# schwanbeck/YSMR

Hardware: AMD Instinct MI355X
Metric: frames/sec detect+link, 1228x922 ~500 blobs, 1/2/4/8 GPU; HBM GB/s %peak (higher is better)
Workload: dtype u8 image / f32 threshold+geometry / f64 link; 1 GPU; 1228x922 stream, ~500 blobs, detect+link end to end (BASELINE configs[2], the configuration the metric is quoted on); detect_batch=248, channels=1, streams=1, parallelism=1 stream/GPU x1, tracks_alive=508, ids_issued=796

## Files before the change

### ysmr_amd/csrc/batch_link.h

```cpp
#pragma once

#include "tracker_plan.h"

constexpr unsigned BL_FLAG = 0xFFFFu, BL_SPLIT = 0xFFFEu;

constexpr int BG_THREADS = 256, BG_PER = 10;
constexpr int BG_CAND = 32;
static_assert(BG_THREADS == 4 * 64 && BL_OVF <= 64, "k_bgrid's second pass: quadrant w of overflow entry `lane` on wave w");
static_assert(BG_THREADS * BG_PER >= FUSED_MAX_DET, "k_bgrid keeps a frame's detections in registers, BG_PER per thread");

__device__ __forceinline__ void bl_rect_list(int cx, int cy, float ax, float bx, float ay, float by, float e, int G, int m, float cell,
                                             float inv, const unsigned short *start16, const float2 *xy, unsigned short *list8,
                                             unsigned short *cand)
{
    float u2 = 3.0e38f;
    int ju = 0;
    auto far2 = [&](int a, int b) {
        for (int j = a; j < b; ++j) {
            const float2 d = xy[j];
            const float dx = fmaxf(fabsf(d.x - ax), fabsf(d.x - bx)), dy = fmaxf(fabsf(d.y - ay), fabsf(d.y - by));
            const float v = dx * dx + dy * dy;
            ju = v < u2 ? j : ju;
            u2 = fminf(u2, v);
        }
    };
    for (int r = 0; r < G; ++r) {
        const int xl = max(cx - r, 0), xh = min(cx + r, G - 1);
        for (int y = max(cy - r, 0); y <= min(cy + r, G - 1); ++y) {
            if (y == cy - r || y == cy + r) far2(start16[y * G + xl], start16[y * G + xh + 1]);
            else {
                if (cx - r >= 0) far2(start16[y * G + cx - r], start16[y * G + cx - r + 1]);
                if (cx + r < G) far2(start16[y * G + cx + r], start16[y * G + cx + r + 1]);
            }
        }
        const float reach = (float)(r + 1) * cell;
        if (u2 <= reach * reach) break;
    }
    const float T = sqrtf(u2) * 1.0001f + 1.0f, T2 = T * T;
    const int rho = min((int)((T + e) * inv) + 2, G);
    int n = 0;
    for (int y = max(cy - rho, 0); y <= min(cy + rho, G - 1); ++y) {
        const int a = start16[y * G + max(cx - rho, 0)], b = start16[y * G + min(cx + rho, G - 1) + 1];
        for (int j = a; j < b; ++j) {
            const float2 d = xy[j];
            const float dx = fmaxf(fmaxf(ax - d.x, d.x - bx), 0.f), dy = fmaxf(fmaxf(ay - d.y, d.y - by), 0.f);
            if (dx * dx + dy * dy <= T2) {
                if (n < BG_CAND) cand[n * BG_THREADS] = (unsigned short)j;
                ++n;
            }
        }
    }
    int kept = 0;
    const float2 du = xy[ju];
    const float ua = ax - du.x, ub = bx - du.x, va = ay - du.y, vb = by - du.y;
    const float eps = 1.00003f, beta = 0.6f;
    const float u0 = (ua * ua + va * va) * eps + beta, u1 = (ub * ub + va * va) * eps + beta;
    const float u2c = (ua * ua + vb * vb) * eps + beta, u3 = (ub * ub + vb * vb) * eps + beta;
    if (n <= BG_CAND)
        for (int i = 0; i < n; ++i) {
            const int ji = cand[i * BG_THREADS];
            const float2 di = xy[ji];
            const float xa = ax - di.x, xb = bx - di.x, ya = ay - di.y, yb = by - di.y;
            const float s0 = xa * xa + ya * ya, s1 = xb * xb + ya * ya, s2 = xa * xa + yb * yb, s3 = xb * xb + yb * yb;
            bool beaten = ji != ju && s0 > u0 && s1 > u1 && s2 > u2c && s3 > u3;
            for (int k = 0; k < n && !beaten; k += 4) {
                float2 dk[4];
#pragma unroll
                for (int u = 0; u < 4; ++u) dk[u] = xy[cand[min(k + u, n - 1) * BG_THREADS]];
#pragma unroll
                for (int u = 0; u < 4; ++u) {
                    const float ka = ax - dk[u].x, kb = bx - dk[u].x, la = ay - dk[u].y, lb = by - dk[u].y;
                    beaten = beaten || (k + u < n && k + u != i && s0 > (ka * ka + la * la) * eps + beta && s1 > (kb * kb + la * la) * eps + beta &&
                                        s2 > (ka * ka + lb * lb) * eps + beta && s3 > (kb * kb + lb * lb) * eps + beta);
                }
            }
            if (!beaten) {
                if (kept < BL_LIST) list8[kept] = (unsigned short)ji;
                ++kept;
            }
        }
    if (n > BG_CAND || kept > BL_LIST) list8[0] = (unsigned short)BL_FLAG;
    else
        for (int k = kept; k < BL_LIST; ++k) list8[k] = (unsigned short)m;
}
__device__ __forceinline__ void bl_cell_list(int c, int G, int m, float x0, float y0, float cell, float inv, const unsigned short *start16,
                                             const float2 *xy, unsigned short *list16, unsigned short *cand)
{
    const int cx = c % G, cy = c / G;
    const float e = 4e-3f + 2e-4f * cell;
    const float ax = x0 + (float)cx * cell - e, bx = x0 + (float)(cx + 1) * cell + e;
    const float ay = y0 + (float)cy * cell - e, by = y0 + (float)(cy + 1) * cell + e;
    bl_rect_list(cx, cy, ax, bx, ay, by, e, G, m, cell, inv, start16, xy, list16 + c * BL_LIST, cand);
}
__device__ __forceinline__ void bl_quad_list(int c, int q, int G, int m, float x0, float y0, float cell, float inv, const unsigned short *start16,
                                             const float2 *xy, unsigned short *list8, unsigned short *cand)
{
    const int cx = c % G, cy = c / G;
    const float e = 4e-3f + 2e-4f * cell;
    const float hx = (float)cx + 0.5f * (float)(q & 1), hy = (float)cy + 0.5f * (float)(q >> 1);
    const float ax = x0 + hx * cell - e, bx = x0 + (hx + 0.5f) * cell + e;
    const float ay = y0 + hy * cell - e, by = y0 + (hy + 0.5f) * cell + e;
    bl_rect_list(cx, cy, ax, bx, ay, by, e, G, m, cell, inv, start16, xy, list8, cand);
}

template <bool D3>
__device__ __forceinline__ void bl_bin_frame(const float *__restrict__ det_all, const double *__restrict__ third_all,
                                             const int32_t *__restrict__ det_count, int max_det, char *grid, unsigned grid_stride)
{
    extern __shared__ __attribute__((aligned(16))) uint32_t s_out[];
    __shared__ int s_cnt[64 * 64];
    __shared__ float s_red[4][4];
    __shared__ int s_wave_sum[4];
    const int f = blockIdx.x, tid = threadIdx.x, lane = tid & 63, w = tid >> 6;
    __shared__ unsigned short s_cand[BG_CAND][BG_THREADS];
    __shared__ unsigned short s_crowded[BL_OVF];
    __shared__ int s_crowded_n;
    __shared__ int s_any_crowded;
    __shared__ int s_wide;
    const float *det = det_all + (size_t)f * max_det * 5;
    int m = det_count[f];
    m = m < 0 ? 0 : (m > max_det ? max_det : m);
    const int G = bl_grid_n(m), cells = G * G;
    unsigned short *start16 = reinterpret_cast<unsigned short *>(s_out + 16);
    float2 *xy = reinterpret_cast<float2 *>(s_out + 16 + bl_start_dwords(G));
    unsigned short *items = reinterpret_cast<unsigned short *>(s_out + 16 + bl_start_dwords(G) + 2 * bl_mp(m));
    unsigned short *list16 = reinterpret_cast<unsigned short *>(s_out + bl_list_off(m));
    float *z32 = reinterpret_cast<float *>(s_out + bl_list_off(m));
    double *z64 = nullptr;
    if constexpr (D3) z64 = reinterpret_cast<double *>(grid + (size_t)grid_stride * f + 4 * (size_t)bl3_lds_dwords_max(max_det));
    float x[BG_PER], y[BG_PER];
    double z[BG_PER];
    bool wide = false;
#pragma unroll
    for (int k = 0; k < BG_PER; ++k) {
        const int j = tid + k * BG_THREADS;
        x[k] = j < m ? det[(size_t)j * 5] : 0.f;
        y[k] = j < m ? det[(size_t)j * 5 + 1] : 0.f;
        if constexpr (D3) {
            z[k] = j < m ? (third_all + (size_t)f * max_det)[j] : 0.0;
            wide = wide || !(fabs(z[k]) < 4096.0);
        }
    }
    for (int c = tid; c < cells; c += BG_THREADS) s_cnt[c] = 0;
    if constexpr (D3) { if (tid == 0) s_wide = 0; }
    float lo_x = 3.0e38f, lo_y = 3.0e38f, hi_x = -3.0e38f, hi_y = -3.0e38f;
#pragma unroll
    for (int k = 0; k < BG_PER; ++k)
        if (tid + k * BG_THREADS < m) { lo_x = fminf(lo_x, x[k]); hi_x = fmaxf(hi_x, x[k]); lo_y = fminf(lo_y, y[k]); hi_y = fmaxf(hi_y, y[k]); }
#pragma unroll
    for (int d = 32; d >= 1; d >>= 1) {
        lo_x = fminf(lo_x, __shfl_xor(lo_x, d)); hi_x = fmaxf(hi_x, __shfl_xor(hi_x, d));
        lo_y = fminf(lo_y, __shfl_xor(lo_y, d)); hi_y = fmaxf(hi_y, __shfl_xor(hi_y, d));
    }
    if (lane == 0) { s_red[0][w] = lo_x; s_red[1][w] = hi_x; s_red[2][w] = lo_y; s_red[3][w] = hi_y; }
    __syncthreads();
    if constexpr (D3) { if (wide) s_wide = 1; }
    lo_x = s_red[0][0]; hi_x = s_red[1][0]; lo_y = s_red[2][0]; hi_y = s_red[3][0];
    for (int k = 1; k < 4; ++k) {
        lo_x = fminf(lo_x, s_red[0][k]); hi_x = fmaxf(hi_x, s_red[1][k]);
        lo_y = fminf(lo_y, s_red[2][k]); hi_y = fmaxf(hi_y, s_red[3][k]);
    }
    if (m == 0) { lo_x = lo_y = 0.f; hi_x = hi_y = 1.f; }
    const float extent = fmaxf(fmaxf(hi_x - lo_x, hi_y - lo_y), 1.0f);
    const float cell = extent / (float)(G - 2), inv = 1.0f / cell;
    const float x0 = lo_x - cell, y0 = lo_y - cell;
    if (tid < 16) s_out[tid] = 0;
    __syncthreads();
    if (tid == 0) {
        float *h = reinterpret_cast<float *>(s_out);
        h[0] = x0; h[1] = y0; h[2] = cell; h[3] = inv;
        s_out[4] = (uint32_t)G; s_out[5] = (uint32_t)m; s_out[6] = !D3 && bl_has_lists(m) ? BL_LIST : 0;
        if constexpr (D3) s_out[7] = (uint32_t)s_wide;
    }
    int cell_of[BG_PER];
#pragma unroll
    for (int k = 0; k < BG_PER; ++k) {
        int cx = (int)floorf((x[k] - x0) * inv), cy = (int)floorf((y[k] - y0) * inv);
        cx = cx < 0 ? 0 : (cx > G - 1 ? G - 1 : cx);
        cy = cy < 0 ? 0 : (cy > G - 1 ? G - 1 : cy);
        cell_of[k] = cy * G + cx;
        if (tid + k * BG_THREADS < m) atomicAdd(&s_cnt[cell_of[k]], 1);
    }
    __syncthreads();
    const int K = cells / BG_THREADS;
    int local[16], sum = 0;
#pragma unroll
    for (int k = 0; k < 16; ++k)
        if (k < K) { local[k] = sum; sum += s_cnt[tid * K + k]; }
    int incl = sum;
#pragma unroll
    for (int d = 1; d < 64; d <<= 1) { const int o = __shfl_up(incl, d); if (lane >= d) incl += o; }
    if (lane == 63) s_wave_sum[w] = incl;
    __syncthreads();
    int before = incl - sum;
    for (int k = 0; k < w; ++k) before += s_wave_sum[k];
#pragma unroll
    for (int k = 0; k < 16; ++k)
        if (k < K) {
            const int at = before + local[k];
            s_cnt[tid * K + k] = at;
            start16[tid * K + k] = (unsigned short)at;
        }
    if (tid == BG_THREADS - 1) { start16[cells] = (unsigned short)m; start16[cells + 1] = 0; }
    for (int j = m + tid; j < bl_mp(m); j += BG_THREADS) {
        xy[j] = make_float2(1.0e30f, 1.0e30f); items[j] = 0;
        if constexpr (D3) { z32[j] = 0.f; z64[j] = 0.0; }
    }
    __syncthreads();
#pragma unroll
    for (int k = 0; k < BG_PER; ++k) {
        const int j = tid + k * BG_THREADS;
        if (j < m) {
            const int at = atomicAdd(&s_cnt[cell_of[k]], 1);
            items[at] = (unsigned short)j;
            xy[at] = make_float2(x[k], y[k]);
            if constexpr (D3) { z32[at] = (float)z[k]; z64[at] = z[k]; }
        }
    }
    if (!D3 && bl_has_lists(m)) {
        for (int i = tid; i < BL_OVF * 4 * BL_LIST / 2; i += BG_THREADS) s_out[bl_ovf_off(m) + i] = 0;
        if (tid == 0) s_any_crowded = 0;
    }
    __syncthreads();
    if constexpr (!D3) {
        unsigned short *ovf16 = reinterpret_cast<unsigned short *>(s_out + bl_ovf_off(m));
        if (bl_has_lists(m) && m > 0) {
            for (int c = tid; c < cells; c += BG_THREADS) {
                bl_cell_list(c, G, m, x0, y0, cell, inv, start16, xy, list16, &s_cand[0][tid]);
                if (list16[c * BL_LIST] == BL_FLAG) s_any_crowded = 1;
            }
            __syncthreads();
        }
        if (bl_has_lists(m) && m > 0 && s_any_crowded) {
            int mine = 0;
#pragma unroll
            for (int k = 0; k < 16; ++k)
                if (k < K) mine += list16[(tid * K + k) * BL_LIST] == BL_FLAG;
            int inc2 = mine;
#pragma unroll
            for (int d = 1; d < 64; d <<= 1) { const int o = __shfl_up(inc2, d); if (lane >= d) inc2 += o; }
            if (lane == 63) s_wave_sum[w] = inc2;
            __syncthreads();
            int at = inc2 - mine;
            for (int k = 0; k < w; ++k) at += s_wave_sum[k];
            if (mine)
                for (int k = 0; k < K; ++k)
                    if (list16[(tid * K + k) * BL_LIST] == BL_FLAG) {
                        if (at < BL_OVF) s_crowded[at] = (unsigned short)(tid * K + k);
                        ++at;
                    }
            if (tid == BG_THREADS - 1) s_crowded_n = min(at, BL_OVF);
            __syncthreads();
            const int entries = s_crowded_n;
            if (lane < entries)
                bl_quad_list(s_crowded[lane], w, G, m, x0, y0, cell, inv, start16, xy, ovf16 + (4 * lane + w) * BL_LIST, &s_cand[0][tid]);
            __syncthreads();
            if (tid < entries) {
                bool fits = true;
                for (int q = 0; q < 4; ++q) fits = fits && ovf16[(4 * tid + q) * BL_LIST] != BL_FLAG;
                if (fits) reinterpret_cast<uint32_t *>(list16)[s_crowded[tid] * (BL_LIST / 2)] = BL_SPLIT | ((uint32_t)tid << 16);
            }
            __syncthreads();
        }
    }
    uint4 *out = reinterpret_cast<uint4 *>(grid + (size_t)grid_stride * f);
    const uint4 *img = reinterpret_cast<const uint4 *>(s_out);
    for (int i = tid; i < (D3 ? bl3_lds_dwords(m) : bl_grid_dwords(m)) / 4; i += BG_THREADS) out[i] = img[i];
}

__global__ __launch_bounds__(BG_THREADS) void k_bgrid(const float *__restrict__ det_all, const int32_t *__restrict__ det_count,
                                                      int max_det, char *grid, unsigned grid_stride)
{
    bl_bin_frame<false>(det_all, nullptr, det_count, max_det, grid, grid_stride);
}

struct BlSeat {
    double s0x[BL_NF], s1x[BL_NF], s0y[BL_NF], s1y[BL_NF];
    double w[BL_NF], xa[BL_NF], xb[BL_NF];
    double px, py;
    float info[3];
    int id, gone, len, mode, rank;
    bool alive;
};

__device__ __forceinline__ void bl_seat_blank(BlSeat &S)
{
#pragma unroll
    for (int f = 0; f < BL_NF; ++f) { S.s0x[f] = S.s1x[f] = S.s0y[f] = S.s1y[f] = 0.0; S.w[f] = S.xa[f] = S.xb[f] = 0.0; }
    S.px = S.py = 0.0;
    S.info[0] = S.info[1] = S.info[2] = 0.f;
    S.id = S.gone = S.len = S.mode = S.rank = 0;
    S.alive = false;
}

__device__ __forceinline__ void bl_seat_load(BlSeat &S, const BatchDev &bd, int at)
{
    const size_t sc = (size_t)bd.seat_cap;
    const double *p = bd.f64 + at;
#pragma unroll
    for (int f = 0; f < BL_NF; ++f) { S.w[f] = p[sc * f]; S.xa[f] = p[sc * (BL_NF + f)]; S.xb[f] = p[sc * (2 * BL_NF + f)]; }
    S.px = p[sc * (3 * BL_NF)];
    S.py = p[sc * (3 * BL_NF + 1)];
#pragma unroll
    for (int f = 0; f < BL_NF; ++f) {
        const double *q = p + sc * (3 * BL_NF + 2 + 4 * f);
        S.s0x[f] = q[0]; S.s1x[f] = q[sc]; S.s0y[f] = q[2 * sc]; S.s1y[f] = q[3 * sc];
    }
#pragma unroll
    for (int k = 0; k < 3; ++k) S.info[k] = bd.f32[sc * k + at];
    S.id = bd.i32[at]; S.gone = bd.i32[sc + at]; S.len = bd.i32[2 * sc + at]; S.mode = bd.i32[3 * sc + at];
    S.rank = bd.i32[4 * sc + at];
}

__device__ __forceinline__ void bl_seat_store(const BlSeat &S, const BatchDev &bd, int at)
{
    const size_t sc = (size_t)bd.seat_cap;
    double *p = bd.f64 + at;
#pragma unroll
    for (int f = 0; f < BL_NF; ++f) { p[sc * f] = S.w[f]; p[sc * (BL_NF + f)] = S.xa[f]; p[sc * (2 * BL_NF + f)] = S.xb[f]; }
    p[sc * (3 * BL_NF)] = S.px;
    p[sc * (3 * BL_NF + 1)] = S.py;
#pragma unroll
    for (int f = 0; f < BL_NF; ++f) {
        double *q = p + sc * (3 * BL_NF + 2 + 4 * f);
        q[0] = S.s0x[f]; q[sc] = S.s1x[f]; q[2 * sc] = S.s0y[f]; q[3 * sc] = S.s1y[f];
    }
// ... 1317 lines not shown
    const int span = cap > bd.seat_cap ? cap : bd.seat_cap;
    for (int s = blockIdx.x * blockDim.x + threadIdx.x; s < span; s += gridDim.x * blockDim.x) {
        if (s < cap - n) d.free_slots[s] = cap - 1 - s;
        if (s == 0) *d.n_free = cap - n;
        if (s >= bd.seat_cap || n == 0 || !bd.i32[5 * sc + s]) continue;
        const int r = bd.i32[4 * sc + s];
        const double *p = bd.f64 + s;
        double *hist = d.hist + (size_t)r * 2 * L;
        for (int e = 0; e < L && e < BL_HB - 1; ++e) {
            const double2 v = bd.ring[(size_t)((head - 1 - e) & (BL_HB - 1)) * sc + s];
            hist[2 * e] = v.x; hist[2 * e + 1] = v.y;
        }
        double *rec = d.rec + (size_t)r * d.rec_stride;
        rec[0] = __longlong_as_double((long long)(unsigned int)bd.i32[2 * sc + s]);
        rec[1] = __longlong_as_double((long long)(unsigned int)bd.i32[3 * sc + s]);
        for (int f = 0; f < nf && f < BL_NF; ++f) {
            rec[2 + f] = p[sc * f];
            rec[2 + nf + f] = p[sc * (BL_NF + f)];
            rec[2 + 2 * nf + f] = p[sc * (2 * BL_NF + f)];
        }
        d.pos[r] = p[sc * (3 * BL_NF)];
        d.pos[cap + r] = p[sc * (3 * BL_NF + 1)];
        if (seat3) pos3[r] = seat3[s];
        for (int k = 0; k < 3; ++k) d.info[k * cap + r] = bd.f32[sc * k + s];
        d.id[r] = bd.i32[s];
        d.order[r] = r;
        d.gone[r] = bd.i32[sc + s];
        d.row_gone[r] = bd.i32[sc + s];
    }
}

__global__ void k_peek_batch(TrackerDev t, BatchDev bd, int32_t *ids, double *xy, int32_t *gone, int32_t *n_out)
{
    const size_t sc = (size_t)bd.seat_cap;
    const int s = blockIdx.x * blockDim.x + threadIdx.x;
    const int n = *t.n_tracks;
    if (s == 0 && n_out) *n_out = n;
    if (s >= bd.seat_cap || n == 0 || !bd.i32[5 * sc + s]) return;
    const int i = bd.i32[4 * sc + s];
    if (ids) ids[i] = bd.i32[s];
    if (xy) { xy[2 * i] = bd.f64[sc * (3 * BL_NF) + s]; xy[2 * i + 1] = bd.f64[sc * (3 * BL_NF + 1) + s]; }
    if (gone) gone[i] = bd.i32[sc + s];
}

__global__ void k_peek_third_batch(TrackerDev t, BatchDev bd, const double *seat3, double *third)
{
    const size_t sc = (size_t)bd.seat_cap;
    const int s = blockIdx.x * blockDim.x + threadIdx.x;
    if (s >= bd.seat_cap || *t.n_tracks == 0 || !bd.i32[5 * sc + s]) return;
    third[bd.i32[4 * sc + s]] = seat3[s];
}


__global__ __launch_bounds__(BG_THREADS) void k_bgrid3(const float *__restrict__ det_all, const double *__restrict__ third_all,
                                                       const int32_t *__restrict__ det_count, int max_det, char *grid, unsigned grid_stride)
{
    bl_bin_frame<true>(det_all, third_all, det_count, max_det, grid, grid_stride);
}

struct Bl3Seat {
    double px, py, pz;
    float info[3];
    int id, gone, rank;
    bool alive;
};

struct BlKernArgs3 {
    TrackerDev t;
    BatchDev bd;
    const float *det_all;
    const double *third_all;
    const int32_t *det_count;
    int batch, frame0;
    ysmr_row *rows;
    long long rows_capacity;
    long long *row_count;
    double *seat3;
};
typedef const __attribute__((address_space(4))) BlKernArgs3 *BlKernArgs3Ptr;
__device__ __forceinline__ BlKernArgs3Ptr bl_kernargs3()
{
    BlKernArgs3Ptr p = (BlKernArgs3Ptr)__builtin_amdgcn_kernarg_segment_ptr();
    asm volatile("" : "+s"(p));
    return p;
}

__global__ __launch_bounds__(BL_THREADS) void k_batch3(BlKernArgs3 ka)
{
    const TrackerDev &t = ka.t;
    const BatchDev &bd = ka.bd;
    const int32_t *__restrict__ det_count = ka.det_count;
    const int batch = ka.batch;
    long long *row_count = ka.row_count;
    __shared__ BlShared sh;
    const int tid = threadIdx.x, lane = tid & 63, wave = __builtin_amdgcn_readfirstlane(tid >> 6);
    const unsigned long long below = (1ull << lane) - 1ull;
    int md = t.max_det, mdp = bl_md_padded(md);
    int bufw = bl3_lds_dwords_max(md);
    auto key_at = [&](int k) { return bl_lds + k * mdp; };
    auto cid_at = [&]() { return bl_u32(6 * mdp); };
    auto buf_off = [&](int p) { return 7 * mdp + p * bufw; };
    auto tab_off = [&]() { return 7 * mdp + 2 * bufw; };
    const int seats = min(t.capacity, BL_THREADS);
    const int gone_max = (int)floor(t.max_gone);

    int n = *t.n_tracks, next_id = *t.next_id;
    long long base = *row_count;
    for (int f = tid; f < batch; f += BL_THREADS) {
        int m = det_count[f];
        if (m > md) { m = md; atomicOr(t.err, ERR_DET_CLAMPED); }
// ... 256 lines not shown
```

### ysmr_amd/csrc/track.hip

```cpp
#include "common.h"
#include "set_order.h"
#include "tracker_plan.h"
#include <algorithm>
#include <cmath>
#include <cstdlib>
#include <cstring>
#include <vector>

struct DetGrid {
    const int *start;
    const int *items;
    const float *hdr;
    const float2 *xy;
};

namespace plan = tracker_plan;

struct ysmr_tracker {
    TrackerDev d;
    TrackerDev d1;
    int par = 0;
    plan::Config cfg;
    plan::Caps caps;
    int dims = 2;
// ... 1702 lines not shown

}

int ysmr::fused_max_det() { return FUSED_MAX_DET; }

#ifndef BL_PAUSE_TICKS_N
#define BL_PAUSE_TICKS_N 1200
#endif
constexpr int BL_PAUSE_TICKS = BL_PAUSE_TICKS_N;
__global__ __launch_bounds__(64) void k_pause(int ticks)
{
    unsigned long long t0, t;
    asm volatile("s_memrealtime %0\n\ts_waitcnt lgkmcnt(0)" : "=s"(t0)::"memory");
    do {
        __builtin_amdgcn_s_sleep(8);
        asm volatile("s_memrealtime %0\n\ts_waitcnt lgkmcnt(0)" : "=s"(t)::"memory");
    } while (t - t0 < (unsigned long long)ticks);
}

extern "C" {

int ysmr_gsff_gains(double fps, int n_min, double n_max, int n_f, int32_t *n_i_out, double *gains_out)
{
    int n_i[YSMR_MAX_FILTERS];
    if (plan::Status s = plan::horizons(fps, n_min, n_max, n_f, n_i)) return plan_fail(s);
    if (!n_i_out) return ysmr::fail(YSMR_ERR_ARG, "n_i_out must not be NULL");
    size_t off = 0;
    for (int i = 0; i < n_f; ++i) {
        n_i_out[i] = n_i[i];
        if (gains_out) plan::closed_form_gain(n_i[i], gains_out + off);
        off += 4 * (size_t)n_i[i];
    }
    return YSMR_OK;
}

static void clear_refused(plan::Caps &q)
{
#ifdef YSMR_TUNING
    if (const char *mode_env = getenv("YSMR_LINK_MODE")) {
        if (!strcmp(mode_env, "split")) q.frame = false;
        if (strcmp(mode_env, "batch")) q.batch = false;
        if (!strcmp(mode_env, "waves")) q.lanes = false;
    }
#endif
    if (q.frame) {
        const void *variants[4] = {(const void *)k_frame<float, 3>, (const void *)k_frame<double, 3>,
                                   (const void *)k_frame<float, YSMR_MAX_FILTERS>, (const void *)k_frame<double, YSMR_MAX_FILTERS>};
        for (const void *fn : variants)
            if (hipFuncSetAttribute(fn, hipFuncAttributeMaxDynamicSharedMemorySize, (int)q.frame_lds) != hipSuccess) q.frame = false;
    }
    if (q.frame && q.batch &&
        hipFuncSetAttribute((const void *)k_batch, hipFuncAttributeMaxDynamicSharedMemorySize, (int)q.batch_lds) != hipSuccess)
        q.batch = false;
}

static int destroy_failed(ysmr_tracker *t, int rc)
{
    if (t->block) (void)hipFree(t->block);
    if (t->grid_block) (void)hipFree(t->grid_block);
    delete t;
    return rc;
}

int ysmr_tracker_create(double max_disappeared, double fps, int n_min, double n_max, int n_f, int use_gsff,
                        int capacity, int max_det, const double *gains_host, ysmr_tracker **out)
{
    if (!out) return ysmr::fail(YSMR_ERR_ARG, "out must not be NULL");
    *out = nullptr;
    ysmr_tracker *t = new ysmr_tracker();
    const plan::Config &c = t->cfg;
    if (plan::Status s = plan::configure(max_disappeared, fps, n_min, n_max, n_f, use_gsff, capacity, max_det, gains_host, t->cfg,
                                         t->gains_host))
        return destroy_failed(t, plan_fail(s));
    plan::Caps &q = t->caps = plan::qualifies(c);
    t->block_bytes = plan::carve_state(nullptr, c, t->d, t->d1, t->bd, t->pos3);
    hipError_t e = hipMalloc(&t->block, t->block_bytes);
    if (e != hipSuccess) {
        t->block = nullptr;
        return destroy_failed(t, ysmr::fail(YSMR_ERR_HIP, "hipMalloc(%zu) failed: %s", t->block_bytes, hipGetErrorString(e)));
    }
    clear_refused(q);
    plan::carve_state(t->block, c, t->d, t->d1, t->bd, t->pos3);
    t->d.gone_by_row = t->d1.gone_by_row = q.frame ? 1 : 0;
    const plan::Link own = t->link();
    const bool lane_bank = own == plan::Link::batch || own == plan::Link::lanes;
    const plan::GridBlocks g = plan::grid_blocks(q, max_det);
    if (g.blocks) {
        const size_t bytes = g.per_frame * BL_MAX_BATCH * g.blocks;
        e = hipMalloc(&t->grid_block, bytes + 256);
        if (e != hipSuccess) t->grid_block = nullptr;
        if (e == hipSuccess && lane_bank) {
            t->bgains_dev = reinterpret_cast<const BlGains *>((char *)t->grid_block + bytes);
            e = hipMemcpy((void *)t->bgains_dev, &c.bgains, sizeof(BlGains), hipMemcpyHostToDevice);
        }
        if (e != hipSuccess) return destroy_failed(t, ysmr::fail(YSMR_ERR_HIP, "hipMalloc(%zu) failed: %s", bytes, hipGetErrorString(e)));
        t->grid_frames = BL_MAX_BATCH;
        t->bd.grid = (char *)t->grid_block;
        t->bd.grid_stride = (unsigned)g.per_frame;
    }
    e = hipMemset(t->block, 0, t->block_bytes);
    if (e == hipSuccess && own == plan::Link::lanes)
        e = hipMemset(t->bd.i32, 0xFF, sizeof(int) * (size_t)t->bd.seat_cap);
    if (e == hipSuccess && c.gain_total)
        e = hipMemcpy((void *)t->d.gains, t->gains_host.data(), sizeof(double) * c.gain_total, hipMemcpyHostToDevice);
    if (e != hipSuccess) return destroy_failed(t, ysmr::fail(YSMR_ERR_HIP, "tracker state initialisation failed: %s", hipGetErrorString(e)));
    *out = t;
// ... 142 lines not shown
int ysmr_debug_seat_events(ysmr_tracker *t, int *events_out, int *moved_out)
{
    int w[3];
    if (!events_out || !moved_out) return ysmr::fail(YSMR_ERR_ARG, "events_out and moved_out must be set");
    if (int rc = seat_words(t, w)) return rc;
    *events_out = w[0]; *moved_out = w[1];
    return YSMR_OK;
}
int ysmr_debug_track_waves(ysmr_tracker *t, int *out)
{
    int w[3];
    if (!out) return ysmr::fail(YSMR_ERR_ARG, "out must be set");
    if (int rc = seat_words(t, w)) return rc;
    *out = w[2];
    return YSMR_OK;
}
int ysmr_debug_ring_zero_line(ysmr_tracker *t, long long *nonzero)
{
    if (!t || !nonzero) return ysmr::fail(YSMR_ERR_ARG, "tracker handle and nonzero must be set");
    std::vector<unsigned long long> line(2 * (size_t)t->bd.seat_cap);
    hipError_t e = hipDeviceSynchronize();
    if (e == hipSuccess)
        e = hipMemcpy(line.data(), t->bd.ring + (size_t)BL_HB * t->bd.seat_cap, sizeof(double2) * (size_t)t->bd.seat_cap, hipMemcpyDeviceToHost);
    if (e != hipSuccess) return ysmr::fail(YSMR_ERR_HIP, "ring read failed: %s", hipGetErrorString(e));
    *nonzero = 0;
    for (unsigned long long w : line) *nonzero += w != 0;
    return YSMR_OK;
}

int ysmr_debug_read_grid_block(ysmr_tracker *t, int slot, int frame, void *out, size_t bytes)
{
    if (!t || !out) return ysmr::fail(YSMR_ERR_ARG, "tracker handle and out must be set");
    if (t->link() != plan::Link::batch) return ysmr::fail(YSMR_ERR_STATE, "the handle has no batch link: no grid blocks");
    if (slot < 0 || slot > 1 || t->prepared[slot].batch <= 0 || frame < 0 || frame >= t->prepared[slot].batch || bytes > t->bd.grid_stride)
        return ysmr::fail(YSMR_ERR_ARG, "slot 0 or 1 with a prepared batch, a frame of that batch, at most %u bytes", t->bd.grid_stride);
    hipError_t e = hipDeviceSynchronize();
    if (e == hipSuccess)
        e = hipMemcpy(out, t->bd.grid + ((size_t)slot * BL_MAX_BATCH + (size_t)frame) * t->bd.grid_stride, bytes, hipMemcpyDeviceToHost);
    return e == hipSuccess ? YSMR_OK : ysmr::fail(YSMR_ERR_HIP, "grid block read failed: %s", hipGetErrorString(e));
}

static BatchDev batch_dev(const ysmr_tracker *t, int block)
{
    BatchDev bd = t->bd;
    if (t->dims == 3) { bd.grid = (char *)t->grid3_block; bd.grid_stride = t->grid3_stride; }
    bd.grid += (size_t)block * BL_MAX_BATCH * bd.grid_stride;
    return bd;
}

static void bin_batch(const ysmr_tracker *t, hipStream_t st, const float *det, const double *third, const int32_t *count, int batch,
                      const BatchDev &bd)
{
    if (t->dims == 3)
        hipLaunchKernelGGL(k_bgrid3, dim3(batch), dim3(BG_THREADS), 4 * (size_t)bl3_lds_dwords_max(t->d.max_det), st, det, third, count,
                           t->d.max_det, bd.grid, bd.grid_stride);
    else
        hipLaunchKernelGGL(k_bgrid, dim3(batch), dim3(BG_THREADS), bd.grid_stride, st, det, count, t->d.max_det, bd.grid, bd.grid_stride);
}

static int tracker_prepare(ysmr_tracker *t, hipStream_t st, const float *det_dev, const double *third_dev, const int32_t *det_count_dev,
                           int batch, int slot)
{
    if (!plan::is_batch(t->link()) || batch > BL_MAX_BATCH) return YSMR_OK;
    bin_batch(t, st, det_dev, third_dev, det_count_dev, batch, batch_dev(t, slot));
    YSMR_LAUNCH_CHECK();
    t->prepared[slot] = ysmr_tracker::Prepared{det_dev, det_count_dev, third_dev, batch};
    return YSMR_OK;
}

int ysmr_tracker_prepare(ysmr_tracker *t, void *stream, const float *det_dev, const int32_t *det_count_dev, int batch, int slot)
{
    if (!t) return ysmr::fail(YSMR_ERR_ARG, "tracker handle is NULL");
    if (!det_dev || !det_count_dev || batch <= 0 || slot < 0 || slot > 1)
        return ysmr::fail(YSMR_ERR_ARG, "det_dev, det_count_dev must be set, batch > 0, slot 0 or 1");
    if (t->dims != 2) return YSMR_OK;
    return tracker_prepare(t, (hipStream_t)stream, det_dev, nullptr, det_count_dev, batch, slot);
}

int ysmr_tracker_prepare3(ysmr_tracker *t, void *stream, const float *det_dev, const double *third_dev, const int32_t *det_count_dev,
                          int batch, int slot)
{
    if (!t) return ysmr::fail(YSMR_ERR_ARG, "tracker handle is NULL");
    if (!det_dev || !third_dev || !det_count_dev || batch <= 0 || slot < 0 || slot > 1)
        return ysmr::fail(YSMR_ERR_ARG, "det_dev, third_dev, det_count_dev must be set, batch > 0, slot 0 or 1");
    if (t->dims != 3) return ysmr::fail(YSMR_ERR_STATE, "ysmr_tracker_prepare3 needs a 3-D handle (ysmr_tracker_dimensions)");
    return tracker_prepare(t, (hipStream_t)stream, det_dev, third_dev, det_count_dev, batch, slot);
}

static int tracker_update(ysmr_tracker *t, hipStream_t st, const void *det_dev, int det_is_f64, const double *third_dev, int m,
                          const int32_t *m_dev, int32_t frame_index, ysmr_row *rows_dev, int32_t *n_rows_dev, int32_t *claim_col_dev,
                          int32_t *n_before_dev, int32_t *new_cols_dev, int32_t *n_new_dev)
{
    if (int rc = state_to_std(t, st)) return rc;
    FrameArgs a;
    a.det = det_dev; a.f64 = det_is_f64 != 0; a.third = third_dev;
    a.m = m; a.m_dev = m_dev; a.frame = frame_index;
    a.rows = rows_dev; a.rows_capacity = t->d.capacity;
    a.n_rows = n_rows_dev; a.claim = claim_col_dev; a.n_before = n_before_dev; a.new_cols = new_cols_dev; a.n_new = n_new_dev;
    return launch_frame(t, st, a);
}

int ysmr_tracker_update(ysmr_tracker *t, void *stream, const void *det_dev, int det_is_f64, int m,
                        const int32_t *m_dev, int32_t frame_index, ysmr_row *rows_dev, int32_t *n_rows_dev,
                        int32_t *claim_col_dev, int32_t *n_before_dev, int32_t *new_cols_dev, int32_t *n_new_dev)
{
    if (!t) return ysmr::fail(YSMR_ERR_ARG, "tracker handle is NULL");
    if (m < 0 && !m_dev) return ysmr::fail(YSMR_ERR_ARG, "m < 0 requires m_dev");
// ... 162 lines not shown
```

### ysmr_amd/csrc/tracker_plan.h

```cpp
#pragma once
#include <cmath>
#include <cstddef>
#include <cstdint>
#include <cstring>
#include <vector>

#include "hd.h"

#ifndef __HIPCC__
struct alignas(16) double2 { double x, y; };
#endif

#define YSMR_MAX_FILTERS 8

struct TrackerDev {
    int *n_tracks, *next_id, *err, *n_free;
    int *order, *gone;
    int *row_arg;
    double *row_min;
    long long *row_base;
    int capacity, max_det, n_f, use_gsff, hist_cap, table_cap, gain_total, gone_by_row;
    int gains_decoupled;
    double max_gone, lik_min;
    int n_i[YSMR_MAX_FILTERS];
// ... 44 lines not shown
    int seat_cap;
};

struct BlGains { double alpha[BL_NF][2], beta[BL_NF][2]; };
constexpr int GRID_N = 128;
constexpr int GRID_CELLS = GRID_N * GRID_N;
YSMR_HD inline size_t grid_bytes_per_frame(int max_det)
{
    return (sizeof(int) * (GRID_CELLS + 64) + sizeof(int) * (size_t)max_det + 64 + 2 * sizeof(float) * (size_t)max_det + 255) / 256 * 256;
}

constexpr int FRAME_THREADS = 256;
constexpr int FRAME_TABLE = 4096;
YSMR_HD inline size_t frame_lds_bytes(int cap, int max_det, int gain_total)
{
    return 8 * ((size_t)gain_total + max_det) + 4 * ((size_t)max_det + 2 * (size_t)cap + 16) + 2 * 2 * FRAME_TABLE + 64;
}

constexpr int TRACKER_MAX_SIZE = 65536;
constexpr int FUSED_MAX_DET = 2456;
constexpr size_t FRAME_LDS_LIMIT = 150 * 1024;
constexpr double FUSED_MAX_GONE = 32000.0;
constexpr size_t LINK_LDS_LIMIT = 140 * 1024;
constexpr size_t BL_LDS_LIMIT = 160 * 1024;

constexpr int BL_LIST = 8;
constexpr int BL_OVF = 8;
YSMR_HD inline int bl_grid_n(int m) { return m <= 128 ? 16 : (m <= 600 ? 32 : (m <= 1300 ? 48 : 64)); }
YSMR_HD inline bool bl_has_lists(int m) { return bl_grid_n(m) <= 32; }
YSMR_HD inline int bl_start_dwords(int G) { return ((G * G + 2) / 2 + 3) / 4 * 4; }
YSMR_HD inline int bl_pad8(int m) { return (m + 7) / 8 * 8; }
YSMR_HD inline int bl_mp(int m) { return bl_pad8(m + 1); }
YSMR_HD inline int bl_list_off(int m)
{
    return 16 + bl_start_dwords(bl_grid_n(m)) + 2 * bl_mp(m) + bl_mp(m) / 2;
}
YSMR_HD inline int bl_ovf_off(int m)
{
    return bl_list_off(m) + bl_grid_n(m) * bl_grid_n(m) * BL_LIST / 2;
}
YSMR_HD inline int bl_grid_dwords(int m)
{
    const int raw = bl_has_lists(m) ? bl_ovf_off(m) + BL_OVF * 4 * BL_LIST / 2 : bl_list_off(m);
    return (raw + 255) / 256 * 256;
}
YSMR_HD inline int bl_grid_dwords_max(int max_det)
{
    int most = bl_grid_dwords(max_det);
    const int steps[4] = {128, 600, 1300, max_det};
    for (int k = 0; k < 4; ++k)
        if (steps[k] <= max_det && bl_grid_dwords(steps[k]) > most) most = bl_grid_dwords(steps[k]);
    return most;
}

struct BlShared {
    int cnt[BL_MAX_BATCH];
    int used[2];
    int n_dead[2];
    int tie[2];
    int dead_id[2][BL_THREADS];
    int wave_cnt[2][BL_WAVES];
    int set_state[2];
    int top;
    long long rows_then;
};

YSMR_HD inline int bl_md_padded(int max_det) { return (max_det + 3) / 4 * 4; }
YSMR_HD inline size_t bl_lds_bytes(int max_det)
{
    return 2 * 4 * (size_t)bl_grid_dwords_max(max_det) + (3 * 8 + 4) * (size_t)bl_md_padded(max_det) + 4 * BL_TABLE + 64;
}
YSMR_HD inline size_t bl_lds_total(int max_det) { return bl_lds_bytes(max_det) + (sizeof(BlShared) + 15) / 16 * 16; }

YSMR_HD inline int bl3_lds_dwords(int m) { return (bl_list_off(m) + bl_mp(m) + 255) / 256 * 256; }
YSMR_HD inline int bl3_lds_dwords_max(int max_det) { return bl3_lds_dwords(max_det); }
YSMR_HD inline size_t bl3_grid_stride(int max_det)
{
    return 4 * (size_t)bl3_lds_dwords_max(max_det) + (8 * (size_t)bl_mp(max_det) + 1023) / 1024 * 1024;
}
YSMR_HD inline size_t bl3_lds_bytes(int max_det)
{
    return 2 * 4 * (size_t)bl3_lds_dwords_max(max_det) + (3 * 8 + 4) * (size_t)bl_md_padded(max_det) + 4 * BL_TABLE + 64;
}
YSMR_HD inline size_t bl3_lds_total(int max_det) { return bl3_lds_bytes(max_det) + (sizeof(BlShared) + 15) / 16 * 16; }

namespace tracker_plan {

enum class Bad { none, size, filters, fps, horizons, horizon_max };
struct Status {
    Bad what = Bad::none;
    int a = 0, b = 0, c = 0;
    double x = 0.0;
    explicit operator bool() const { return what != Bad::none; }
};

inline Status horizons(double fps, int n_min, double n_max, int n_f, int *n_i)
{
    if (n_f < 1 || n_f > YSMR_MAX_FILTERS) return Status{Bad::filters, YSMR_MAX_FILTERS, n_f};
    if (!(fps > 0)) return Status{Bad::fps};
    double top = n_max > 0 ? n_max : fps;
    double p = (top - n_min) / n_f;
    for (int i = 1; i <= n_f; ++i) n_i[i - 1] = (int)(n_min + p * i);
    for (int i = 0; i < n_f; ++i)
        if (n_i[i] < 1 || (i && n_i[i] <= n_i[i - 1])) return Status{Bad::horizons, n_min, n_f, 0, top};
    return Status{};
}
// ... 99 lines not shown
    std::memcpy(d0.n_i, c.n_i, sizeof(d0.n_i));
    std::memcpy(d0.gain_off, c.gain_off, sizeof(d0.gain_off));
    auto word = [](int *s, int k) { return s ? s + k : nullptr; };
    auto scalars = [&](TrackerDev &q) {
        int *s = a.take<int>(16);
        q.n_tracks = s; q.next_id = word(s, 1); q.n_free = word(s, 3);
        q.row_base = reinterpret_cast<long long *>(word(s, 8));
        return s;
    };
    int *scal = scalars(d0);
    d0.err = word(scal, 2);
    bd.head = word(scal, 12);
    d0.order = a.take<int>(cap); d0.free_slots = a.take<int>(cap);
    d0.id = a.take<int>(cap); d0.gone = a.take<int>(cap);
    d0.pos = a.take<double>(2 * cap); d0.info = a.take<float>(3 * cap);
    pos3 = a.take<double>(cap);
    d0.hist = a.take<double>(2 * cap * c.hist_cap);
    d0.rec = a.take<double>((size_t)c.rec_stride * cap);
    d0.gains = a.take<double>(c.gain_total ? c.gain_total : 1);
    d0.unused = a.take<int>(md);
    d0.row_min = a.take<double>(cap); d0.row_arg = a.take<int>(cap); d0.row_gone = a.take<int>(cap);
    d0.dead = a.take<int>(cap);
    d0.new_cols = a.take<int>(md); d0.set_table = a.take<int>(2 * (size_t)c.table_cap);
    d0.link_key = a.take<unsigned long long>(md); d0.link_row = a.take<int>(md);
    d0.link_claim = a.take<int>(cap); d0.claim_slot = a.take<int>(cap); d0.claim_row = a.take<int>(cap);
    d1 = d0;
    scalars(d1);
    d1.order = a.take<int>(cap); d1.gone = a.take<int>(cap);
    d1.row_min = a.take<double>(cap); d1.row_arg = a.take<int>(cap);
    const size_t seat_cap = c.capacity > BL_THREADS ? cap : (size_t)BL_THREADS;
    bd.ring = a.take<double2>((BL_HB + 1) * seat_cap);
    bd.f64 = a.take<double>(BL_SF64 * seat_cap); bd.f32 = a.take<float>(3 * seat_cap);
    bd.i32 = a.take<int>(6 * seat_cap);
    bd.seat_cap = (int)seat_cap;
    bd.grid = nullptr; bd.grid_stride = 0;
    return a.at;
}

enum class Link {
    frame,
    waves,
    lanes,
    batch,
    batch3,
};

struct Caps {
    bool frame;
    bool lanes;
    bool batch;
    bool batch3;
    bool link_lds;
    size_t frame_lds, batch_lds, batch3_lds, link_lds_bytes;
};

inline Caps qualifies(const Config &c)
{
    Caps q{};
    q.frame_lds = frame_lds_bytes(c.capacity, c.max_det, c.gain_total);
    q.batch_lds = bl_lds_bytes(c.max_det);
    q.batch3_lds = bl3_lds_bytes(c.max_det);
    q.link_lds_bytes = 12 * (size_t)c.max_det;
    q.frame = q.frame_lds <= FRAME_LDS_LIMIT && c.max_det <= FUSED_MAX_DET && c.max_gone < FUSED_MAX_GONE;
    q.lanes = c.n_f <= BL_NF && c.hist_cap <= BL_HB && (!c.use_gsff || (c.gains_decoupled && c.gains_affine));
    q.batch = q.frame && q.lanes && c.capacity <= BL_THREADS && bl_lds_total(c.max_det) <= BL_LDS_LIMIT;
    q.batch3 = q.frame && !c.use_gsff && c.capacity <= BL_THREADS && bl3_lds_total(c.max_det) <= BL_LDS_LIMIT;
    q.link_lds = q.link_lds_bytes <= LINK_LDS_LIMIT;
    return q;
}

inline Link link_of(const Caps &q, int dims, int link_mode)
{
    if (dims == 3) {
        if (q.frame && q.batch3 && link_mode == 2) return Link::batch3;
        return q.frame ? Link::frame : Link::waves;
    }
    if (q.frame && q.batch && link_mode != 1) return Link::batch;
    if (q.frame) return Link::frame;
    return q.lanes ? Link::lanes : Link::waves;
}
inline bool is_batch(Link l) { return l == Link::batch || l == Link::batch3; }
inline bool uses_det_grids(Link l, int dims) { return dims == 2 && (l == Link::waves || l == Link::lanes); }

struct GridBlocks { size_t per_frame; int blocks; };
inline GridBlocks grid_blocks(const Caps &q, int max_det)
{
    const Link l = link_of(q, 2, 0);
    if (l == Link::batch) return GridBlocks{(size_t)bl_grid_dwords_max(max_det) * 4, 3};
    if (l == Link::frame) return GridBlocks{0, 0};
    return GridBlocks{grid_bytes_per_frame(max_det), 1};
}

}
```

Measured before the change: 292,400 frames/s.

## Run 2D grid binning with 1024 threads and prefilter candidate dominance

Templates the grid-binning kernel on thread count and launches the 2D variant with 1024 threads instead of 256, so per-frame cell list construction and the overflow quadrant pass spread across sixteen waves. The overflow quadrant work is redistributed evenly across waves, and static LDS grows with the wider candidate buffer, with a new LDS capacity check and a dynamic-shared-memory attribute. The dominance test in the cell-list builder first drops candidates already beaten by the nearest-far point, then runs the pairwise check only on survivors. The larger block raises LDS use per block and may reduce occupancy or disable the batch path for large max_det.

```diff
diff --git a/ysmr_amd/csrc/batch_link.h b/ysmr_amd/csrc/batch_link.h
--- a/ysmr_amd/csrc/batch_link.h
+++ b/ysmr_amd/csrc/batch_link.h
@@ -4,11 +4,13 @@
 
 constexpr unsigned BL_FLAG = 0xFFFFu, BL_SPLIT = 0xFFFEu;
 
-constexpr int BG_THREADS = 256, BG_PER = 10;
-constexpr int BG_CAND = 32;
-static_assert(BG_THREADS == 4 * 64 && BL_OVF <= 64, "k_bgrid's second pass: quadrant w of overflow entry `lane` on wave w");
-static_assert(BG_THREADS * BG_PER >= FUSED_MAX_DET, "k_bgrid keeps a frame's detections in registers, BG_PER per thread");
-
+constexpr int bg_per(int threads) { return (2560 + threads - 1) / threads; }
+static_assert(BG_THREADS % 64 == 0 && BG_THREADS / 64 <= 16 && (BL_OVF * 4) % (BG_THREADS / 64) == 0 && BL_OVF * 4 / (BG_THREADS / 64) <= 64,
+              "k_bgrid's second pass: the (entry, quadrant) items in equal shares on the waves' first lanes");
+static_assert(BG_THREADS * bg_per(BG_THREADS) >= FUSED_MAX_DET && BG3_THREADS * bg_per(BG3_THREADS) >= FUSED_MAX_DET,
+              "k_bgrid keeps a frame's detections in registers, bg_per per thread");
+
+template <int STRIDE>
 __device__ __forceinline__ void bl_rect_list(int cx, int cy, float ax, float bx, float ay, float by, float e, int G, int m, float cell,
                                              float inv, const unsigned short *start16, const float2 *xy, unsigned short *list8,
                                              unsigned short *cand)
@@ -45,32 +47,42 @@
             const float2 d = xy[j];
             const float dx = fmaxf(fmaxf(ax - d.x, d.x - bx), 0.f), dy = fmaxf(fmaxf(ay - d.y, d.y - by), 0.f);
             if (dx * dx + dy * dy <= T2) {
-                if (n < BG_CAND) cand[n * BG_THREADS] = (unsigned short)j;
+                if (n < BG_CAND) cand[n * STRIDE] = (unsigned short)j;
                 ++n;
             }
         }
     }
-    int kept = 0;
+    int kept = 0, n1 = 0;
     const float2 du = xy[ju];
     const float ua = ax - du.x, ub = bx - du.x, va = ay - du.y, vb = by - du.y;
     const float eps = 1.00003f, beta = 0.6f;
     const float u0 = (ua * ua + va * va) * eps + beta, u1 = (ub * ub + va * va) * eps + beta;
     const float u2c = (ua * ua + vb * vb) * eps + beta, u3 = (ub * ub + vb * vb) * eps + beta;
-    if (n <= BG_CAND)
+    if (n <= BG_CAND) {
         for (int i = 0; i < n; ++i) {
-            const int ji = cand[i * BG_THREADS];
+            const int ji = cand[i * STRIDE];
             const float2 di = xy[ji];
             const float xa = ax - di.x, xb = bx - di.x, ya = ay - di.y, yb = by - di.y;
             const float s0 = xa * xa + ya * ya, s1 = xb * xb + ya * ya, s2 = xa * xa + yb * yb, s3 = xb * xb + yb * yb;
-            bool beaten = ji != ju && s0 > u0 && s1 > u1 && s2 > u2c && s3 > u3;
-            for (int k = 0; k < n && !beaten; k += 4) {
+            if (!(ji != ju && s0 > u0 && s1 > u1 && s2 > u2c && s3 > u3)) {
+                cand[n1 * STRIDE] = (unsigned short)ji;
+                ++n1;
+            }
+        }
+        for (int i = 0; i < n1; ++i) {
+            const int ji = cand[i * STRIDE];
+            const float2 di = xy[ji];
+            const float xa = ax - di.x, xb = bx - di.x, ya = ay - di.y, yb = by - di.y;
+            const float s0 = xa * xa + ya * ya, s1 = xb * xb + ya * ya, s2 = xa * xa + yb * yb, s3 = xb * xb + yb * yb;
+            bool beaten = false;
+            for (int k = 0; k < n1 && !beaten; k += 4) {
                 float2 dk[4];
 #pragma unroll
-                for (int u = 0; u < 4; ++u) dk[u] = xy[cand[min(k + u, n - 1) * BG_THREADS]];
+                for (int u = 0; u < 4; ++u) dk[u] = xy[cand[min(k + u, n1 - 1) * STRIDE]];
 #pragma unroll
                 for (int u = 0; u < 4; ++u) {
                     const float ka = ax - dk[u].x, kb = bx - dk[u].x, la = ay - dk[u].y, lb = by - dk[u].y;
-                    beaten = beaten || (k + u < n && k + u != i && s0 > (ka * ka + la * la) * eps + beta && s1 > (kb * kb + la * la) * eps + beta &&
+                    beaten = beaten || (k + u < n1 && k + u != i && s0 > (ka * ka + la * la) * eps + beta && s1 > (kb * kb + la * la) * eps + beta &&
                                         s2 > (ka * ka + lb * lb) * eps + beta && s3 > (kb * kb + lb * lb) * eps + beta);
                 }
             }
@@ -79,10 +91,12 @@
                 ++kept;
             }
         }
+    }
     if (n > BG_CAND || kept > BL_LIST) list8[0] = (unsigned short)BL_FLAG;
     else
         for (int k = kept; k < BL_LIST; ++k) list8[k] = (unsigned short)m;
 }
+template <int STRIDE>
 __device__ __forceinline__ void bl_cell_list(int c, int G, int m, float x0, float y0, float cell, float inv, const unsigned short *start16,
                                              const float2 *xy, unsigned short *list16, unsigned short *cand)
 {
@@ -90,8 +104,9 @@
     const float e = 4e-3f + 2e-4f * cell;
     const float ax = x0 + (float)cx * cell - e, bx = x0 + (float)(cx + 1) * cell + e;
     const float ay = y0 + (float)cy * cell - e, by = y0 + (float)(cy + 1) * cell + e;
-    bl_rect_list(cx, cy, ax, bx, ay, by, e, G, m, cell, inv, start16, xy, list16 + c * BL_LIST, cand);
-}
+    bl_rect_list<STRIDE>(cx, cy, ax, bx, ay, by, e, G, m, cell, inv, start16, xy, list16 + c * BL_LIST, cand);
+}
+template <int STRIDE>
 __device__ __forceinline__ void bl_quad_list(int c, int q, int G, int m, float x0, float y0, float cell, float inv, const unsigned short *start16,
                                              const float2 *xy, unsigned short *list8, unsigned short *cand)
 {
@@ -100,23 +115,26 @@
     const float hx = (float)cx + 0.5f * (float)(q & 1), hy = (float)cy + 0.5f * (float)(q >> 1);
     const float ax = x0 + hx * cell - e, bx = x0 + (hx + 0.5f) * cell + e;
     const float ay = y0 + hy * cell - e, by = y0 + (hy + 0.5f) * cell + e;
-    bl_rect_list(cx, cy, ax, bx, ay, by, e, G, m, cell, inv, start16, xy, list8, cand);
-}
-
-template <bool D3>
+    bl_rect_list<STRIDE>(cx, cy, ax, bx, ay, by, e, G, m, cell, inv, start16, xy, list8, cand);
+}
+
+template <bool D3, int THREADS>
 __device__ __forceinline__ void bl_bin_frame(const float *__restrict__ det_all, const double *__restrict__ third_all,
                                              const int32_t *__restrict__ det_count, int max_det, char *grid, unsigned grid_stride)
 {
     extern __shared__ __attribute__((aligned(16))) uint32_t s_out[];
     __shared__ int s_cnt[64 * 64];
-    __shared__ float s_red[4][4];
-    __shared__ int s_wave_sum[4];
+    constexpr int PER = bg_per(THREADS), WAVES = THREADS / 64;
+    __shared__ float s_red[4][WAVES];
+    __shared__ int s_wave_sum[WAVES];
     const int f = blockIdx.x, tid = threadIdx.x, lane = tid & 63, w = tid >> 6;
-    __shared__ unsigned short s_cand[BG_CAND][BG_THREADS];
+    __shared__ unsigned short s_cand[BG_CAND][THREADS];
     __shared__ unsigned short s_crowded[BL_OVF];
     __shared__ int s_crowded_n;
     __shared__ int s_any_crowded;
     __shared__ int s_wide;
+    static_assert(D3 || sizeof(s_cnt) + sizeof(s_red) + sizeof(s_wave_sum) + sizeof(s_cand) + sizeof(s_crowded) + 3 * sizeof(int) + 64 <=
+                            BG_LDS_STATIC, "tracker_plan.h: k_bgrid's static LDS");
     const float *det = det_all + (size_t)f * max_det * 5;
     int m = det_count[f];
     m = m < 0 ? 0 : (m > max_det ? max_det : m);
@@ -128,12 +146,12 @@
     float *z32 = reinterpret_cast<float *>(s_out + bl_list_off(m));
     double *z64 = nullptr;
     if constexpr (D3) z64 = reinterpret_cast<double *>(grid + (size_t)grid_stride * f + 4 * (size_t)bl3_lds_dwords_max(max_det));
-    float x[BG_PER], y[BG_PER];
-    double z[BG_PER];
+    float x[PER], y[PER];
+    double z[PER];
     bool wide = false;
 #pragma unroll
-    for (int k = 0; k < BG_PER; ++k) {
-        const int j = tid + k * BG_THREADS;
+    for (int k = 0; k < PER; ++k) {
+        const int j = tid + k * THREADS;
         x[k] = j < m ? det[(size_t)j * 5] : 0.f;
         y[k] = j < m ? det[(size_t)j * 5 + 1] : 0.f;
         if constexpr (D3) {
@@ -141,12 +159,12 @@
             wide = wide || !(fabs(z[k]) < 4096.0);
         }
     }
-    for (int c = tid; c < cells; c += BG_THREADS) s_cnt[c] = 0;
+    for (int c = tid; c < cells; c += THREADS) s_cnt[c] = 0;
     if constexpr (D3) { if (tid == 0) s_wide = 0; }
     float lo_x = 3.0e38f, lo_y = 3.0e38f, hi_x = -3.0e38f, hi_y = -3.0e38f;
 #pragma unroll
-    for (int k = 0; k < BG_PER; ++k)
-        if (tid + k * BG_THREADS < m) { lo_x = fminf(lo_x, x[k]); hi_x = fmaxf(hi_x, x[k]); lo_y = fminf(lo_y, y[k]); hi_y = fmaxf(hi_y, y[k]); }
+    for (int k = 0; k < PER; ++k)
+        if (tid + k * THREADS < m) { lo_x = fminf(lo_x, x[k]); hi_x = fmaxf(hi_x, x[k]); lo_y = fminf(lo_y, y[k]); hi_y = fmaxf(hi_y, y[k]); }
 #pragma unroll
     for (int d = 32; d >= 1; d >>= 1) {
         lo_x = fminf(lo_x, __shfl_xor(lo_x, d)); hi_x = fmaxf(hi_x, __shfl_xor(hi_x, d));
@@ -156,7 +174,7 @@
     __syncthreads();
     if constexpr (D3) { if (wide) s_wide = 1; }
     lo_x = s_red[0][0]; hi_x = s_red[1][0]; lo_y = s_red[2][0]; hi_y = s_red[3][0];
-    for (int k = 1; k < 4; ++k) {
+    for (int k = 1; k < WAVES; ++k) {
         lo_x = fminf(lo_x, s_red[0][k]); hi_x = fmaxf(hi_x, s_red[1][k]);
         lo_y = fminf(lo_y, s_red[2][k]); hi_y = fmaxf(hi_y, s_red[3][k]);
     }
@@ -172,21 +190,22 @@
         s_out[4] = (uint32_t)G; s_out[5] = (uint32_t)m; s_out[6] = !D3 && bl_has_lists(m) ? BL_LIST : 0;
         if constexpr (D3) s_out[7] = (uint32_t)s_wide;
     }
-    int cell_of[BG_PER];
-#pragma unroll
-    for (int k = 0; k < BG_PER; ++k) {
+    int cell_of[PER];
+#pragma unroll
+    for (int k = 0; k < PER; ++k) {
         int cx = (int)floorf((x[k] - x0) * inv), cy = (int)floorf((y[k] - y0) * inv);
         cx = cx < 0 ? 0 : (cx > G - 1 ? G - 1 : cx);
         cy = cy < 0 ? 0 : (cy > G - 1 ? G - 1 : cy);
         cell_of[k] = cy * G + cx;
-        if (tid + k * BG_THREADS < m) atomicAdd(&s_cnt[cell_of[k]], 1);
+        if (tid + k * THREADS < m) atomicAdd(&s_cnt[cell_of[k]], 1);
     }
     __syncthreads();
-    const int K = cells / BG_THREADS;
+    const int K = (cells + THREADS - 1) / THREADS;
+    auto owns = [&](int c) { return THREADS <= 256 || c < cells; };
     int local[16], sum = 0;
 #pragma unroll
     for (int k = 0; k < 16; ++k)
-        if (k < K) { local[k] = sum; sum += s_cnt[tid * K + k]; }
+        if (k < K && owns(tid * K + k)) { local[k] = sum; sum += s_cnt[tid * K + k]; }
     int incl = sum;
 #pragma unroll
     for (int d = 1; d < 64; d <<= 1) { const int o = __shfl_up(incl, d); if (lane >= d) incl += o; }
@@ -196,20 +215,20 @@
     for (int k = 0; k < w; ++k) before += s_wave_sum[k];
 #pragma unroll
     for (int k = 0; k < 16; ++k)
-        if (k < K) {
+        if (k < K && owns(tid * K + k)) {
             const int at = before + local[k];
             s_cnt[tid * K + k] = at;
             start16[tid * K + k] = (unsigned short)at;
         }
-    if (tid == BG_THREADS - 1) { start16[cells] = (unsigned short)m; start16[cells + 1] = 0; }
-    for (int j = m + tid; j < bl_mp(m); j += BG_THREADS) {
+    if (tid == THREADS - 1) { start16[cells] = (unsigned short)m; start16[cells + 1] = 0; }
+    for (int j = m + tid; j < bl_mp(m); j += THREADS) {
         xy[j] = make_float2(1.0e30f, 1.0e30f); items[j] = 0;
         if constexpr (D3) { z32[j] = 0.f; z64[j] = 0.0; }
     }
     __syncthreads();
 #pragma unroll
-    for (int k = 0; k < BG_PER; ++k) {
-        const int j = tid + k * BG_THREADS;
+    for (int k = 0; k < PER; ++k) {
+        const int j = tid + k * THREADS;
         if (j < m) {
             const int at = atomicAdd(&s_cnt[cell_of[k]], 1);
             items[at] = (unsigned short)j;
@@ -218,15 +237,15 @@
         }
     }
     if (!D3 && bl_has_lists(m)) {
-        for (int i = tid; i < BL_OVF * 4 * BL_LIST / 2; i += BG_THREADS) s_out[bl_ovf_off(m) + i] = 0;
+        for (int i = tid; i < BL_OVF * 4 * BL_LIST / 2; i += THREADS) s_out[bl_ovf_off(m) + i] = 0;
         if (tid == 0) s_any_crowded = 0;
     }
     __syncthreads();
     if constexpr (!D3) {
         unsigned short *ovf16 = reinterpret_cast<unsigned short *>(s_out + bl_ovf_off(m));
         if (bl_has_lists(m) && m > 0) {
-            for (int c = tid; c < cells; c += BG_THREADS) {
-                bl_cell_list(c, G, m, x0, y0, cell, inv, start16, xy, list16, &s_cand[0][tid]);
+            for (int c = tid; c < cells; c += THREADS) {
+                bl_cell_list<THREADS>(c, G, m, x0, y0, cell, inv, start16, xy, list16, &s_cand[0][tid]);
                 if (list16[c * BL_LIST] == BL_FLAG) s_any_crowded = 1;
             }
             __syncthreads();
@@ -235,7 +254,7 @@
             int mine = 0;
 #pragma unroll
             for (int k = 0; k < 16; ++k)
-                if (k < K) mine += list16[(tid * K + k) * BL_LIST] == BL_FLAG;
+                if (k < K && owns(tid * K + k)) mine += list16[(tid * K + k) * BL_LIST] == BL_FLAG;
             int inc2 = mine;
 #pragma unroll
             for (int d = 1; d < 64; d <<= 1) { const int o = __shfl_up(inc2, d); if (lane >= d) inc2 += o; }
@@ -245,15 +264,18 @@
             for (int k = 0; k < w; ++k) at += s_wave_sum[k];
             if (mine)
                 for (int k = 0; k < K; ++k)
-                    if (list16[(tid * K + k) * BL_LIST] == BL_FLAG) {
+                    if (owns(tid * K + k) && list16[(tid * K + k) * BL_LIST] == BL_FLAG) {
                         if (at < BL_OVF) s_crowded[at] = (unsigned short)(tid * K + k);
                         ++at;
                     }
-            if (tid == BG_THREADS - 1) s_crowded_n = min(at, BL_OVF);
+            if (tid == THREADS - 1) s_crowded_n = min(at, BL_OVF);
             __syncthreads();
             const int entries = s_crowded_n;
-            if (lane < entries)
-                bl_quad_list(s_crowded[lane], w, G, m, x0, y0, cell, inv, start16, xy, ovf16 + (4 * lane + w) * BL_LIST, &s_cand[0][tid]);
+            constexpr int SHARE = BL_OVF * 4 / WAVES;
+            const int item = SHARE * w + lane;
+            if (lane < SHARE && (item >> 2) < entries)
+                bl_quad_list<THREADS>(s_crowded[item >> 2], item & 3, G, m, x0, y0, cell, inv, start16, xy, ovf16 + item * BL_LIST,
+                                      &s_cand[0][tid]);
             __syncthreads();
             if (tid < entries) {
                 bool fits = true;
@@ -265,13 +287,13 @@
     }
     uint4 *out = reinterpret_cast<uint4 *>(grid + (size_t)grid_stride * f);
     const uint4 *img = reinterpret_cast<const uint4 *>(s_out);
-    for (int i = tid; i < (D3 ? bl3_lds_dwords(m) : bl_grid_dwords(m)) / 4; i += BG_THREADS) out[i] = img[i];
+    for (int i = tid; i < (D3 ? bl3_lds_dwords(m) : bl_grid_dwords(m)) / 4; i += THREADS) out[i] = img[i];
 }
 
 __global__ __launch_bounds__(BG_THREADS) void k_bgrid(const float *__restrict__ det_all, const int32_t *__restrict__ det_count,
                                                       int max_det, char *grid, unsigned grid_stride)
 {
-    bl_bin_frame<false>(det_all, nullptr, det_count, max_det, grid, grid_stride);
+    bl_bin_frame<false, BG_THREADS>(det_all, nullptr, det_count, max_det, grid, grid_stride);
 }
 
 struct BlSeat {
@@ -1695,10 +1717,10 @@
 }
 
 
-__global__ __launch_bounds__(BG_THREADS) void k_bgrid3(const float *__restrict__ det_all, const double *__restrict__ third_all,
+__global__ __launch_bounds__(BG3_THREADS) void k_bgrid3(const float *__restrict__ det_all, const double *__restrict__ third_all,
                                                        const int32_t *__restrict__ det_count, int max_det, char *grid, unsigned grid_stride)
 {
-    bl_bin_frame<true>(det_all, third_all, det_count, max_det, grid, grid_stride);
+    bl_bin_frame<true, BG3_THREADS>(det_all, third_all, det_count, max_det, grid, grid_stride);
 }
 
 struct Bl3Seat {
diff --git a/ysmr_amd/csrc/track.hip b/ysmr_amd/csrc/track.hip
--- a/ysmr_amd/csrc/track.hip
+++ b/ysmr_amd/csrc/track.hip
@@ -1778,6 +1778,9 @@
     if (q.frame && q.batch &&
         hipFuncSetAttribute((const void *)k_batch, hipFuncAttributeMaxDynamicSharedMemorySize, (int)q.batch_lds) != hipSuccess)
         q.batch = false;
+    if (q.frame && q.batch &&
+        hipFuncSetAttribute((const void *)k_bgrid, hipFuncAttributeMaxDynamicSharedMemorySize, (int)q.bgrid_lds) != hipSuccess)
+        q.batch = false;
 }
 
 static int destroy_failed(ysmr_tracker *t, int rc)
@@ -2026,7 +2029,7 @@
                       const BatchDev &bd)
 {
     if (t->dims == 3)
-        hipLaunchKernelGGL(k_bgrid3, dim3(batch), dim3(BG_THREADS), 4 * (size_t)bl3_lds_dwords_max(t->d.max_det), st, det, third, count,
+        hipLaunchKernelGGL(k_bgrid3, dim3(batch), dim3(BG3_THREADS), 4 * (size_t)bl3_lds_dwords_max(t->d.max_det), st, det, third, count,
                            t->d.max_det, bd.grid, bd.grid_stride);
     else
         hipLaunchKernelGGL(k_bgrid, dim3(batch), dim3(BG_THREADS), bd.grid_stride, st, det, count, t->d.max_det, bd.grid, bd.grid_stride);
diff --git a/ysmr_amd/csrc/tracker_plan.h b/ysmr_amd/csrc/tracker_plan.h
--- a/ysmr_amd/csrc/tracker_plan.h
+++ b/ysmr_amd/csrc/tracker_plan.h
@@ -120,6 +120,13 @@
         if (steps[k] <= max_det && bl_grid_dwords(steps[k]) > most) most = bl_grid_dwords(steps[k]);
     return most;
 }
+
+constexpr int BG_THREADS = 1024;
+constexpr int BG3_THREADS = 256;
+constexpr int BG_CAND = 32;
+constexpr size_t BG_LDS_STATIC = 4 * 64 * 64 + 2 * (size_t)BG_CAND * BG_THREADS + 512;
+YSMR_HD inline size_t bg_lds_bytes(int max_det) { return 4 * (size_t)bl_grid_dwords_max(max_det); }
+YSMR_HD inline size_t bg_lds_total(int max_det) { return bg_lds_bytes(max_det) + BG_LDS_STATIC; }
 
 struct BlShared {
     int cnt[BL_MAX_BATCH];
@@ -325,6 +332,7 @@
     bool batch3;
     bool link_lds;
     size_t frame_lds, batch_lds, batch3_lds, link_lds_bytes;
+    size_t bgrid_lds;
 };
 
 inline Caps qualifies(const Config &c)
@@ -334,9 +342,11 @@
     q.batch_lds = bl_lds_bytes(c.max_det);
     q.batch3_lds = bl3_lds_bytes(c.max_det);
     q.link_lds_bytes = 12 * (size_t)c.max_det;
+    q.bgrid_lds = bg_lds_bytes(c.max_det);
     q.frame = q.frame_lds <= FRAME_LDS_LIMIT && c.max_det <= FUSED_MAX_DET && c.max_gone < FUSED_MAX_GONE;
     q.lanes = c.n_f <= BL_NF && c.hist_cap <= BL_HB && (!c.use_gsff || (c.gains_decoupled && c.gains_affine));
-    q.batch = q.frame && q.lanes && c.capacity <= BL_THREADS && bl_lds_total(c.max_det) <= BL_LDS_LIMIT;
+    q.batch = q.frame && q.lanes && c.capacity <= BL_THREADS && bl_lds_total(c.max_det) <= BL_LDS_LIMIT &&
+              bg_lds_total(c.max_det) <= BL_LDS_LIMIT;
     q.batch3 = q.frame && !c.use_gsff && c.capacity <= BL_THREADS && bl3_lds_total(c.max_det) <= BL_LDS_LIMIT;
     q.link_lds = q.link_lds_bytes <= LINK_LDS_LIMIT;
     return q;
```

Result: no change. 292,800 frames/s, median of 3 (+0.2%).
